# ForeverFancy/GVFDiffusion

Measured on AMD Instinct MI355X. Metric: 4D frames/sec (800x800x24f, 256k Gaussians) + DiT denoise steps/sec, higher is better.
Workload: dtype f32

## Files before the change

gvfdiffusion_amd/csrc/rast.hip:

```cpp
#include <atomic>
#include <cstdlib>
#include <mutex>
#include <vector>
#include "gvf_common.h"
#include "gvf_sort.h"
#include "../../include/gvf_rast.h"

namespace {

constexpr int PRE_THREADS = 256;
constexpr int NSLAB = 1;
#ifndef GVF_PRE_FB
#define GVF_PRE_FB 4
#endif
constexpr int PRE_FB = GVF_PRE_FB;
#ifndef GVF_PRE_XCD
#define GVF_PRE_XCD 0
#endif
#ifndef GVF_PRE_REC_QUAD
#define GVF_PRE_REC_QUAD 1
#endif
#ifndef GVF_PRE_PREFETCH
#define GVF_PRE_PREFETCH 0
#endif
constexpr int TILE = GVF_TILE;
constexpr int BLEND_THREADS = TILE * TILE;
constexpr int MAX_SH_COEFFS = 16;
constexpr float CONIC_K1 = -0.7213475204444817f;
constexpr float CONIC_K2 = -1.4426950408889634f;
constexpr float CONIC_IK1 = -1.3862943611198906f;
constexpr float CONIC_IK2 = -0.6931471805599453f;
struct SplatChol { float l11, l12, l22, c1, c2; bool ok; };
__device__ __forceinline__ SplatChol splat_cholesky(float x, float y, float ap, float bp, float cp, float tile_x0, float tile_y0) {
    SplatChol r;
    const float m11 = -ap, m12 = -0.5f * bp, m22 = -cp;
    const float il = __builtin_amdgcn_rsqf(m11);
    r.l11 = m11 * il;
    r.l12 = m12 * il;
    const float d = m22 - r.l12 * r.l12;
    r.l22 = __builtin_amdgcn_sqrtf(d);
    r.ok = m11 > 0.0f && d > 0.0f && m11 < __builtin_inff() && d < __builtin_inff();
    if (!r.ok) { r.l11 = 0.f; r.l12 = 0.f; r.l22 = 0.f; }
    const float xr = x - tile_x0, yr = y - tile_y0;
    r.c1 = r.ok ? __builtin_fmaf(r.l11, xr, r.l12 * yr) : 0.f;
    r.c2 = r.ok ? r.l22 * yr : 0.f;
    return r;
}
__device__ __forceinline__ float splat_neg_exponent(float l11, float l12, float l22, float c1, float c2, float px, float py, float lo = 0.0f) {
    const float s1 = __builtin_fmaf(-l11, px, __builtin_fmaf(-l12, py, c1));
    const float s2 = __builtin_fmaf(-l22, py, c2);
    return __builtin_fmaf(s2, s2, __builtin_fmaf(s1, s1, -lo));
}

__constant__ float SH_C0 = 0.28209479177387814f;
__constant__ float SH_C1 = 0.4886025119029199f;
__constant__ float SH_C2[5] = {1.0925484305920792f, -1.0925484305920792f, 0.31539156525252005f,
                               -1.0925484305920792f, 0.5462742152960396f};
__constant__ float SH_C3[7] = {-0.5900435899266435f, 2.890611442640554f, -0.4570457994644658f,
                               0.3731763325901154f, -0.4570457994644658f, 1.445305721320277f,
                               -0.5900435899266435f};

struct PreParams {
    int P, M, deg, H, W, mode;
    int gx, gy;
    float kernel_size, scale_modifier;
    int fused;
    GvfGaussianActivation act;
    int n_delta;
    int upstream_binning;
    int F;
};

__device__ __forceinline__ float act_expf(float x) {
    if (x != x) return x;
    if (x > 88.72283f) return __builtin_inff();
    if (x < -103.97208f) return 0.0f;
    const float kf = x * 1.44269502f + (x < 0.0f ? -0.5f : 0.5f);
    const int k = (int)kf;
    const float t = (float)k;
    float r = __builtin_fmaf(t, -0.693145751953125f, x);
    r = __builtin_fmaf(t, -1.42860677e-6f, r);
    float p = 1.98412698e-4f;
    p = __builtin_fmaf(p, r, 1.38888889e-3f);
    p = __builtin_fmaf(p, r, 8.33333377e-3f);
    p = __builtin_fmaf(p, r, 4.16666679e-2f);
    p = __builtin_fmaf(p, r, 1.66666672e-1f);
    p = __builtin_fmaf(p, r, 0.5f);
    p = __builtin_fmaf(p, r, 1.0f);
    p = __builtin_fmaf(p, r, 1.0f);
    const int k1 = k / 2, k2 = k - k1;
    return (p * __uint_as_float((uint32_t)(k1 + 127) << 23)) * __uint_as_float((uint32_t)(k2 + 127) << 23);
}
__device__ __forceinline__ float act_log1pf(float y) {
    if (!(y >= 5.9604645e-8f)) return y;
    if (y > 3.4028235e38f) return y;
    int k = 0;
    float c = 0.0f, f = y;
    if (y >= 0.41421354f) {
        const float u = 1.0f + y;
        uint32_t iu = __float_as_uint(u) + (0x3f800000u - 0x3f3504f3u);
        k = (int)(iu >> 23) - 127;
        if (k < 25) c = (k >= 2 ? 1.0f - (u - y) : y - (u - 1.0f)) / u;
        iu = (iu & 0x007fffffu) + 0x3f3504f3u;
        f = __uint_as_float(iu) - 1.0f;
    }
    const float s = f / (2.0f + f);
    const float z = s * s, w = z * z;
    const float t1 = w * (0.40000972152f + w * 0.24279078841f);
    const float t2 = z * (0.66666662693f + w * 0.28498786688f);
    const float R = t2 + t1;
    const float hfsq = (0.5f * f) * f;
    const float dk = (float)k;
    float acc = s * (hfsq + R);
    acc = acc + (dk * 9.0580006145e-6f + c);
    acc = acc - hfsq;
    acc = acc + f;
    return acc + dk * 6.9313812256e-1f;
}
#ifdef ACT_ABL_LIBM
#define act_expf expf
#define act_log1pf log1pf
#endif
__device__ __forceinline__ float act_scale(float x, const GvfGaussianActivation& a) {
// ... 193 lines not shown
    return make_float2(sqrtf(tau * cc * inv) * 1.001f + 0.01f, sqrtf(tau * ca * inv) * 1.001f + 0.01f);
}

__device__ __forceinline__ void tight_range(float c, float h, int lo, int hi, int n, int& t0, int& t1) {
    if (h < 0.0f) { t0 = lo; t1 = lo; return; }
    const float a = fminf(fmaxf(ceilf((c - h - (float)(TILE - 1)) / (float)TILE), 0.0f), (float)n);
    const float b = fminf(fmaxf(floorf((c + h) / (float)TILE) + 1.0f, 0.0f), (float)n);
    t0 = max((int)a, lo);
    t1 = min((int)b, hi);
    if (t1 < t0) t1 = t0;
}

__device__ __forceinline__ TileRect tight_rect(TileRect r, float px, float py, float hx, float hy, int gx, int gy) {
    TileRect t;
    tight_range(px, hx, r.x0, r.x1, gx, t.x0, t.x1);
    tight_range(py, hy, r.y0, r.y1, gy, t.y0, t.y1);
    return t;
}

template <bool SHARED>
__global__ __launch_bounds__(PRE_THREADS) void preprocess_kernel(
    PreParams pp, const GvfRastFrame* __restrict__ frames, const float* __restrict__ a0,
    const float* __restrict__ a1, const float* __restrict__ a2, const float* __restrict__ a3,
    const float* __restrict__ sh, const float* __restrict__ colors_precomp,
    const float* __restrict__ cov3D_precomp, const float* __restrict__ delta, float4* __restrict__ splats,
    uint32_t* __restrict__ tiles_touched,
    int32_t* __restrict__ radii, uint32_t* __restrict__ block_sums, uint4* __restrict__ binrec,
    const uint32_t* __restrict__ bin_slot ,
    const float2* __restrict__ zrange ) {
    extern __shared__ __attribute__((aligned(16))) float sh_lds[];
    const int t = threadIdx.x;
    const int P = pp.P, M = pp.M;
    const int nbx = (P + PRE_THREADS - 1) / PRE_THREADS;
    int bx = blockIdx.x, by = blockIdx.y;
    if (GVF_PRE_XCD) {
        const int FY = (pp.F + PRE_FB - 1) / PRE_FB, k = (int)(blockIdx.x >> 3);
        bx = (k / FY) * 8 + (int)(blockIdx.x & 7u);
        by = k - (k / FY) * FY;
        if (bx >= nbx) return;
    }
    const int i = bx * PRE_THREADS + t;

    const int sh_stride = M * 3;
    if (sh != nullptr) {
        const size_t span0 = (size_t)bx * PRE_THREADS * sh_stride;
        const int nvalid = min(PRE_THREADS, P - bx * PRE_THREADS);
        const int total = nvalid * sh_stride;
        const float4* src4 = reinterpret_cast<const float4*>(sh + span0);
        float4* dst4 = reinterpret_cast<float4*>(sh_lds);
        const int n4 = total >> 2;
        for (int k = t; k < n4; k += PRE_THREADS) dst4[k] = src4[k];
        for (int k = (n4 << 2) + t; k < total; k += PRE_THREADS) sh_lds[k] = sh[span0 + k];
    }
    __syncthreads();

  const uint32_t my_slot = (bin_slot != nullptr && i < P) ? bin_slot[i] : (uint32_t)i;
#if GVF_PRE_PREFETCH
  float dnx[14];
  bool dnx_has = false;
  auto fetch_delta = [&](int f_) {
      dnx_has = false;
      if (pp.fused && delta != nullptr && i < P && f_ < pp.F) {
          const int di = frames[f_].delta_index;
          if (di >= 0) {
              const float* d = delta + ((size_t)di * P + i) * 14;
#pragma unroll
              for (int k = 0; k < 14; ++k) dnx[k] = d[k];
              dnx_has = true;
          }
      }
      if (!dnx_has) {
#pragma unroll
          for (int k = 0; k < 14; ++k) dnx[k] = 0.0f;
      }
  };
  fetch_delta(by * PRE_FB);
#endif
  for (int ff = 0; ff < PRE_FB; ++ff) {
    const int f = by * PRE_FB + ff;
    if (f >= pp.F) break;
    const GvfRastFrame* fr = frames + f;
#if GVF_PRE_PREFETCH
    float dcur[14];
#pragma unroll
    for (int k = 0; k < 14; ++k) dcur[k] = dnx[k];
    const bool dcur_has = dnx_has;
    if (ff + 1 < PRE_FB) fetch_delta(f + 1);
#endif
    uint32_t touched = 0;
    int radius_out = 0;
    float4 gA = make_float4(0.f, 0.f, 0.f, 0.f), gB = gA, gC = gA;
    TileRect rect = {0, 0, 0, 0};

    if (i < P) {
        float p[3], s[3], q[4], op, dadd[3] = {0.f, 0.f, 0.f};
        float c6s[6];
        if (SHARED) {
            const float4* r3 = reinterpret_cast<const float4*>(a0) + 4 * ((size_t)fr->reserved[0] * P + i);
            const float4 r0 = r3[0], r1 = r3[1], r2 = r3[2], r3v = r3[3];
            p[0] = r0.x; p[1] = r0.y; p[2] = r0.z; op = r0.w;
            c6s[0] = r1.x; c6s[1] = r1.y; c6s[2] = r1.z; c6s[3] = r1.w; c6s[4] = r2.x; c6s[5] = r2.y;
            dadd[0] = r2.z; dadd[1] = r2.w; dadd[2] = r3v.x;
        } else if (pp.fused) {
#if GVF_PRE_PREFETCH
            ActGaussian g = activate_vals(i, pp.act, a0, a1, a2, a3, dcur, dcur_has);
#else
            const int di = fr->delta_index;
            const float* d = (delta != nullptr && di >= 0) ? delta + ((size_t)di * P + i) * 14 : nullptr;
            ActGaussian g = activate_one(i, pp.act, a0, a1, a2, a3, d);
#endif
#pragma unroll
            for (int k = 0; k < 3; ++k) { p[k] = g.p[k]; s[k] = g.s[k]; dadd[k] = g.drgb[k]; }
#pragma unroll
            for (int k = 0; k < 4; ++k) q[k] = g.q[k];
            op = g.op;
        } else {
#pragma unroll
            for (int k = 0; k < 3; ++k) p[k] = a0[3 * (size_t)i + k];
            if (cov3D_precomp == nullptr) {
#pragma unroll
                for (int k = 0; k < 3; ++k) s[k] = a1[3 * (size_t)i + k];
#pragma unroll
                for (int k = 0; k < 4; ++k) q[k] = a2[4 * (size_t)i + k];
            }
            op = a3[i];
        }

        float pv[3];
        xform43(fr->viewmatrix, p, pv);
        bool vis = pv[2] > 0.2f;
        if (vis) {
            float ph[4];
            xform44(fr->projmatrix, p, ph);
            float pw = 1.0f / (ph[3] + 0.0000001f);
            float projx = ph[0] * pw, projy = ph[1] * pw;

            float c6[6];
            if (SHARED) {
#pragma unroll
                for (int k = 0; k < 6; ++k) c6[k] = c6s[k];
            } else if (!pp.fused && cov3D_precomp != nullptr) {
#pragma unroll
                for (int k = 0; k < 6; ++k) c6[k] = cov3D_precomp[6 * (size_t)i + k];
            } else {
                cov3d_from_scale_rot(s, pp.scale_modifier, q, c6);
            }

            const float tanfovx = fr->tanfovx, tanfovy = fr->tanfovy;
            float focal_x = (float)pp.W / (2.0f * tanfovx);
            float focal_y = (float)pp.H / (2.0f * tanfovy);
            float limx = 1.3f * tanfovx, limy = 1.3f * tanfovy;
            float txtz = pv[0] / pv[2], tytz = pv[1] / pv[2];
            float tx = fminf(limx, fmaxf(-limx, txtz)) * pv[2];
            float ty = fminf(limy, fmaxf(-limy, tytz)) * pv[2];
            float tz = pv[2];
            float J00 = focal_x / tz, J02 = -(focal_x * tx) / (tz * tz);
            float J11 = focal_y / tz, J12 = -(focal_y * ty) / (tz * tz);
            float A0[3], A1[3];
// ... 15 lines not shown
            float cyy = B1[0] * A1[0] + B1[1] * A1[1] + B1[2] * A1[2];

            float coef = 1.0f;
            if (pp.mode == GVF_RAST_MODE_MIP) {
                float det0 = fmaxf(1e-6f, cxx * cyy - cxy * cxy);
                float det1 = fmaxf(1e-6f, (cxx + pp.kernel_size) * (cyy + pp.kernel_size) - cxy * cxy);
                coef = sqrtf(det0 / (det1 + 1e-6f) + 1e-6f);
                if (det0 <= 1e-6f || det1 <= 1e-6f) coef = 0.0f;
                cxx += pp.kernel_size;
                cyy += pp.kernel_size;
            } else {
                cxx += 0.3f;
                cyy += 0.3f;
            }
            float det = cxx * cyy - cxy * cxy;
            if (det != 0.0f) {
                float det_inv = 1.f / det;
                float ca = cyy * det_inv, cb = -cxy * det_inv, cc = cxx * det_inv;
                float mid = 0.5f * (cxx + cyy);
                float lam1 = mid + sqrtf(fmaxf(0.1f, mid * mid - det));
                float lam2 = mid - sqrtf(fmaxf(0.1f, mid * mid - det));
                float my_radius = ceilf(3.f * sqrtf(fmaxf(lam1, lam2)));
                float px = ((projx + 1.0f) * (float)pp.W - 1.0f) * 0.5f;
                float py = ((projy + 1.0f) * (float)pp.H - 1.0f) * 0.5f;
                TileRect r = get_rect(px, py, my_radius, pp.gx, pp.gy);
                uint32_t cnt = (uint32_t)((r.x1 - r.x0) * (r.y1 - r.y0));
                if (cnt != 0) {
                    float rgb[3];
                    if (colors_precomp != nullptr) {
                        rgb[0] = colors_precomp[3 * (size_t)i + 0];
                        rgb[1] = colors_precomp[3 * (size_t)i + 1];
                        rgb[2] = colors_precomp[3 * (size_t)i + 2];
                    } else {
                        sh_to_rgb(pp.deg, sh_lds + t * sh_stride, dadd, p, fr->campos, rgb);
                    }
                    radius_out = (int)my_radius;
                    const float2 ext = cull_extent(ca, cb, cc, op * coef);
                    if (!pp.upstream_binning) {
                        r = tight_rect(r, px, py, ext.x, ext.y, pp.gx, pp.gy);
                        cnt = (uint32_t)((r.x1 - r.x0) * (r.y1 - r.y0));
                    }
                    touched = cnt;
                    rect = r;
                    gA = make_float4(px, py, ca * CONIC_K1, cb * CONIC_K2);
                    gB = make_float4(cc * CONIC_K1, op * coef, rgb[0], rgb[1]);
                    gC = make_float4(rgb[2], pv[2], ext.x, ext.y);
                }
            }
        }
        const size_t o = (size_t)f * P + i;
#if defined(PRE_ABL_NOREC)
        if (touched != 0 && gA.x == 12345.678f) splats[4 * o] = gA;
#else
        if (!(GVF_PRE_REC_QUAD && SHARED) && touched != 0) {
            float4* rec = splats + 4 * o;
            rec[0] = gA; rec[1] = gB; rec[2] = gC;
        }
#endif
        if (tiles_touched != nullptr) tiles_touched[o] = touched;
        if (radii != nullptr) {
            const uint32_t* gid_of = SHARED ? reinterpret_cast<const uint32_t*>(a1) : nullptr;
            radii[gid_of != nullptr ? (size_t)f * P + gid_of[i] : o] = radius_out;
        }
        if (binrec != nullptr) {
            uint32_t slab = 0u;
            if (zrange != nullptr) {
                const float2 zr = zrange[f];
                slab = (uint32_t)fminf(fmaxf((gC.y - zr.x) * zr.y, 0.0f), (float)(NSLAB - 1));
            }
#if defined(PRE_ABL_NOBIN)
            if (gC.y == 12345.678f)
#elif defined(PRE_ABL_BINLINEAR)
            binrec[(size_t)f * P + i] = make_uint4((uint32_t)rect.x0 | ((uint32_t)rect.y0 << 16), (uint32_t)rect.x1 | ((uint32_t)rect.y1 << 16), __float_as_uint(gC.y), slab);
            if (false)
#endif
            binrec[(size_t)f * P + my_slot] = make_uint4((uint32_t)rect.x0 | ((uint32_t)rect.y0 << 16),
                                                         (uint32_t)rect.x1 | ((uint32_t)rect.y1 << 16), __float_as_uint(gC.y), slab);
        }
    }

#if !defined(PRE_ABL_NOREC)
    if (GVF_PRE_REC_QUAD && SHARED) {
        const int lj = t & 3;
        float4* qbase = splats + 4 * ((size_t)f * P + (size_t)(i & ~3));
#define GVF_QB(v_, k_) __builtin_bit_cast(float, __builtin_amdgcn_mov_dpp(__builtin_bit_cast(int, (v_)), (k_) * 0x55, 0xF, 0xF, true))
#define GVF_QSTORE(k_)                                                                                          \
        {                                                                                                       \
            const int tk = __builtin_amdgcn_mov_dpp((int)touched, (k_) * 0x55, 0xF, 0xF, true);                 \
            float4 o4;                                                                                          \
            { const float a = GVF_QB(gA.x, k_), b = GVF_QB(gB.x, k_), c = GVF_QB(gC.x, k_); o4.x = lj == 0 ? a : (lj == 1 ? b : (lj == 2 ? c : 0.f)); } \
            { const float a = GVF_QB(gA.y, k_), b = GVF_QB(gB.y, k_), c = GVF_QB(gC.y, k_); o4.y = lj == 0 ? a : (lj == 1 ? b : (lj == 2 ? c : 0.f)); } \
            { const float a = GVF_QB(gA.z, k_), b = GVF_QB(gB.z, k_), c = GVF_QB(gC.z, k_); o4.z = lj == 0 ? a : (lj == 1 ? b : (lj == 2 ? c : 0.f)); } \
            { const float a = GVF_QB(gA.w, k_), b = GVF_QB(gB.w, k_), c = GVF_QB(gC.w, k_); o4.w = lj == 0 ? a : (lj == 1 ? b : (lj == 2 ? c : 0.f)); } \
            if (tk != 0) qbase[4 * (k_) + lj] = o4;                                                             \
        }
        GVF_QSTORE(0) GVF_QSTORE(1) GVF_QSTORE(2) GVF_QSTORE(3)
#undef GVF_QSTORE
#undef GVF_QB
    }
#endif

    if (block_sums != nullptr) {
        const unsigned lane = t & 63, w = t >> 6;
        uint32_t incl = gvf_wave_incl_scan(touched, lane);
        __shared__ uint32_t wsum[PRE_THREADS / GVF_WAVE];
        __syncthreads();
        if (lane == 63) wsum[w] = incl;
        __syncthreads();
        if (t == 0) block_sums[(size_t)f * nbx + bx] = wsum[0] + wsum[1] + wsum[2] + wsum[3];
    }
  }
}

__global__ __launch_bounds__(1024) void scan_sums_kernel(uint32_t* __restrict__ block_sums, int nb, int F,
                                                         uint32_t* __restrict__ frame_base ,
                                                         uint32_t* __restrict__ num_rendered ,
                                                         uint32_t* __restrict__ total_out, uint32_t max_rendered) {
    __shared__ uint32_t wsum[16];
    __shared__ uint32_t carry_s;
    const int t = threadIdx.x;
    const unsigned lane = t & 63, w = t >> 6;
    const int n = nb * F;
    if (t == 0) carry_s = 0;
    __syncthreads();
    for (int base = 0; base < n; base += 1024) {
        int j = base + t;
        uint32_t v = j < n ? block_sums[j] : 0u;
        uint32_t incl = gvf_wave_incl_scan(v, lane);
        if (lane == 63) wsum[w] = incl;
        __syncthreads();
        uint32_t wbase = 0, tot = 0;
        for (unsigned k = 0; k < 16; ++k) { if (k < w) wbase += wsum[k]; tot += wsum[k]; }
        uint32_t carry = carry_s;
        uint32_t excl = carry + wbase + incl - v;
        if (j < n) {
            block_sums[j] = excl;
            if (j % nb == 0) frame_base[j / nb] = excl;
        }
        __syncthreads();
        if (t == 0) carry_s = carry + tot;
        __syncthreads();
    }
    if (t == 0) { frame_base[F] = carry_s; *total_out = carry_s > max_rendered ? 0u : carry_s; }
    __syncthreads();
    for (int f = t; f < F; f += 1024) num_rendered[f] = frame_base[f + 1] - frame_base[f];
}

__global__ __launch_bounds__(PRE_THREADS) void duplicate_kernel(
    int P, int gx, int gy, const float4* __restrict__ splats,
    const uint32_t* __restrict__ tiles_touched, const int32_t* __restrict__ radii_ws,
    const uint32_t* __restrict__ block_base, uint64_t* __restrict__ keys, uint32_t* __restrict__ vals,
    uint32_t max_rendered, int upstream_binning) {
    __shared__ uint32_t wsum[PRE_THREADS / GVF_WAVE];
    const int t = threadIdx.x, f = blockIdx.y;
    const int i = blockIdx.x * PRE_THREADS + t;
    const unsigned lane = t & 63, w = t >> 6;
    const size_t o = (size_t)f * P + i;
    uint32_t touched = i < P ? tiles_touched[o] : 0u;
    uint32_t incl = gvf_wave_incl_scan(touched, lane);
    if (lane == 63) wsum[w] = incl;
    __syncthreads();
    uint32_t wbase = 0;
    for (unsigned k = 0; k < w; ++k) wbase += wsum[k];
// ... 90 lines not shown
        if (j < n) {
            ranges[j] = overflow ? make_uint2(0u, 0u) : make_uint2(run, run + c[k]);
            cursor[j] = run;
            if (!overflow && c[k] > (uint32_t)SORT_SMALL_N) {
                if (c[k] > (uint32_t)SORT_LARGE_N) cls[2 + n + atomicAdd(&cls[1], 1u)] = (uint32_t)j;
                else cls[2 + atomicAdd(&cls[0], 1u)] = (uint32_t)j | (c[k] > (uint32_t)SORT_MEDIUM_N ? 0x80000000u : 0u);
            }
            if (j % per_frame == 0) frame_base[j / per_frame] = run;
        }
        run += c[k];
    }
    if (blockIdx.x == 0 && t == 0) { frame_base[F] = total; *total_out = overflow ? 0u : total; }
}

__global__ void frame_counts_kernel(const uint32_t* __restrict__ frame_base, int F, uint32_t* __restrict__ num_rendered) {
    const int f = blockIdx.x * blockDim.x + threadIdx.x;
    if (f < F) num_rendered[f] = frame_base[f + 1] - frame_base[f];
}

__global__ void frame_zrange_kernel(const GvfRastFrame* __restrict__ frames, int F, const uint32_t* __restrict__ mm,
                                    int fused, GvfGaussianActivation act, float2* __restrict__ zrange) {
    const int f = blockIdx.x * blockDim.x + threadIdx.x;
    if (f >= F) return;
    float lo[3], hi[3];
#pragma unroll
    for (int k = 0; k < 3; ++k) {
        lo[k] = float_unordered(mm[k]); hi[k] = float_unordered(mm[3 + k]);
        if (fused) { lo[k] = lo[k] * act.aabb[3 + k] + act.aabb[k]; hi[k] = hi[k] * act.aabb[3 + k] + act.aabb[k]; }
        if (lo[k] > hi[k]) { const float tmp = lo[k]; lo[k] = hi[k]; hi[k] = tmp; }
    }
    const float* V = frames[f].viewmatrix;
    float zmin = 3.0e38f, zmax = -3.0e38f;
    for (int c = 0; c < 8; ++c) {
        const float p[3] = {(c & 1) ? hi[0] : lo[0], (c & 2) ? hi[1] : lo[1], (c & 4) ? hi[2] : lo[2]};
        const float z = V[2] * p[0] + V[6] * p[1] + V[10] * p[2] + V[14];
        zmin = fminf(zmin, z); zmax = fmaxf(zmax, z);
    }
    zmin = fmaxf(zmin, 0.2f);
    const float ext = fmaxf(zmax - zmin, 1e-6f);
    zrange[f] = make_float2(zmin - 0.02f * ext, (float)NSLAB / (1.04f * ext));
}

constexpr int WIN_MAX = 2048;
constexpr int BIN_SPT = 4;
constexpr int BIN_SLOTS = PRE_THREADS * BIN_SPT;

template <bool SCATTER>
__global__ __launch_bounds__(PRE_THREADS) void bin_kernel(int P, int gx, int gy, const uint4* __restrict__ binrec,
                                                          const uint32_t* __restrict__ order,
                                                          uint32_t* __restrict__ tile_count ,
                                                          uint32_t* __restrict__ cursor ,
                                                          const uint32_t* __restrict__ total,
                                                          uint64_t* __restrict__ payload, int nslab,
                                                          const uint32_t* __restrict__ frame_base, uint32_t* __restrict__ num_rendered) {
    __shared__ uint32_t s_tab[WIN_MAX];
    __shared__ uint32_t s_run[SCATTER ? WIN_MAX : 1];
    __shared__ int s_box[4];
    if (SCATTER && num_rendered != nullptr && blockIdx.x == 0 && threadIdx.x == 0)
        num_rendered[blockIdx.y] = frame_base[blockIdx.y + 1] - frame_base[blockIdx.y];
    if (SCATTER && *total == 0u) return;
    const int t = threadIdx.x, lane = t & 63, f = blockIdx.y;
    if (t == 0) { s_box[0] = 0x7fffffff; s_box[1] = 0x7fffffff; s_box[2] = 0; s_box[3] = 0; }
    int x0[BIN_SPT], y0[BIN_SPT], x1[BIN_SPT], y1[BIN_SPT], sl[BIN_SPT];
    uint64_t key[BIN_SPT];
    int bx0 = 0x7fffffff, by0 = 0x7fffffff, bx1 = 0, by1 = 0;
#pragma unroll
    for (int k = 0; k < BIN_SPT; ++k) {
        const int s = blockIdx.x * BIN_SLOTS + k * PRE_THREADS + t;
        x0[k] = y0[k] = x1[k] = y1[k] = 0; sl[k] = 0; key[k] = 0;
        if (s < P) {
            const uint32_t id = order != nullptr ? order[s] : (uint32_t)s;
            const uint4 br = binrec[(size_t)f * P + s];
            x0[k] = (int)(br.x & 0xffffu); y0[k] = (int)(br.x >> 16);
            x1[k] = (int)(br.y & 0xffffu); y1[k] = (int)(br.y >> 16);
            sl[k] = (int)br.w;
            key[k] = ((uint64_t)br.z << 32) | id;
            if (x1[k] > x0[k] && y1[k] > y0[k]) {
                bx0 = min(bx0, x0[k]); by0 = min(by0, y0[k]); bx1 = max(bx1, x1[k]); by1 = max(by1, y1[k]);
            } else {
                x1[k] = x0[k];
            }
        }
    }
#pragma unroll
    for (int d = 32; d >= 1; d >>= 1) {
        bx0 = min(bx0, __shfl_xor(bx0, d, 64)); by0 = min(by0, __shfl_xor(by0, d, 64));
        bx1 = max(bx1, __shfl_xor(bx1, d, 64)); by1 = max(by1, __shfl_xor(by1, d, 64));
    }
    __syncthreads();
    if (lane == 0 && bx1 > bx0) {
        atomicMin(&s_box[0], bx0); atomicMin(&s_box[1], by0); atomicMax(&s_box[2], bx1); atomicMax(&s_box[3], by1);
    }
    __syncthreads();
    const int wx0 = s_box[0], wy0 = s_box[1], ww = s_box[2] - s_box[0], wh = s_box[3] - s_box[1];
    if (ww <= 0 || wh <= 0) return;
    uint32_t* gtab = (SCATTER ? cursor : tile_count) + (size_t)f * gx * gy * nslab;
    if (ww * wh * nslab <= WIN_MAX) {
        const int area = ww * wh * nslab;
        for (int e = t; e < area; e += PRE_THREADS) { s_tab[e] = 0u; if (SCATTER) s_run[e] = 0u; }
        __syncthreads();
#pragma unroll
        for (int k = 0; k < BIN_SPT; ++k)
            for (int y = y0[k]; y < y1[k]; ++y)
                for (int x = x0[k]; x < x1[k]; ++x) atomicAdd(&s_tab[((y - wy0) * ww + (x - wx0)) * nslab + sl[k]], 1u);
        __syncthreads();
        for (int e = t; e < area; e += PRE_THREADS) {
            const uint32_t c = s_tab[e];
            if (c != 0u) {
                const int wt = e / nslab;
                const int seg = ((wy0 + wt / ww) * gx + wx0 + wt % ww) * nslab + (e - wt * nslab);
                if (SCATTER) s_tab[e] = atomicAdd(&gtab[seg], c);
                else atomicAdd(&gtab[seg], c);
            }
        }
        if (SCATTER) {
            __syncthreads();
#pragma unroll
            for (int k = 0; k < BIN_SPT; ++k)
                for (int y = y0[k]; y < y1[k]; ++y)
                    for (int x = x0[k]; x < x1[k]; ++x) {
                        const int e = ((y - wy0) * ww + (x - wx0)) * nslab + sl[k];
                        payload[s_tab[e] + atomicAdd(&s_run[e], 1u)] = key[k];
                    }
        }
    } else {
#pragma unroll
        for (int k = 0; k < BIN_SPT; ++k)
            for (int y = y0[k]; y < y1[k]; ++y)
                for (int x = x0[k]; x < x1[k]; ++x) {
                    const uint32_t pos = atomicAdd(&gtab[(y * gx + x) * nslab + sl[k]], 1u);
                    if (SCATTER) payload[pos] = key[k];
                }
    }
}

__global__ __launch_bounds__(256) void bbox_kernel(int P, const float* __restrict__ xyz, uint32_t* __restrict__ mm) {
    __shared__ uint32_t s_mm[6];
    if (threadIdx.x < 6) s_mm[threadIdx.x] = threadIdx.x < 3 ? 0xffffffffu : 0u;
    __syncthreads();
    uint32_t lo[3] = {0xffffffffu, 0xffffffffu, 0xffffffffu}, hi[3] = {0u, 0u, 0u};
    for (int i = blockIdx.x * blockDim.x + threadIdx.x; i < P; i += gridDim.x * blockDim.x) {
#pragma unroll
        for (int k = 0; k < 3; ++k) {
            const float v = xyz[3 * (size_t)i + k];
            if (v == v && fabsf(v) < 3.0e38f) {
                const uint32_t o = float_ordered(v);
                lo[k] = min(lo[k], o); hi[k] = max(hi[k], o);
            }
        }
    }
#pragma unroll
    for (int k = 0; k < 3; ++k) {
#pragma unroll
        for (int d = 32; d >= 1; d >>= 1) {
            lo[k] = min(lo[k], (uint32_t)__shfl_xor((int)lo[k], d, 64));
            hi[k] = max(hi[k], (uint32_t)__shfl_xor((int)hi[k], d, 64));
        }
        if ((threadIdx.x & 63) == 0) { atomicMin(&s_mm[k], lo[k]); atomicMax(&s_mm[3 + k], hi[k]); }
    }
    __syncthreads();
    if (threadIdx.x < 3) atomicMin(&mm[threadIdx.x], s_mm[threadIdx.x]);
    else if (threadIdx.x < 6) atomicMax(&mm[threadIdx.x], s_mm[threadIdx.x]);
}

__device__ __forceinline__ uint32_t spread5(uint32_t v) {
    return (v & 1u) | ((v & 2u) << 2) | ((v & 4u) << 4) | ((v & 8u) << 6) | ((v & 16u) << 8);
}

constexpr int MORTON_BINS = 1 << 15;

__device__ __forceinline__ uint32_t morton15(int i, const float* __restrict__ xyz, const uint32_t* __restrict__ mm) {
    uint32_t code = 0;
#pragma unroll
    for (int k = 0; k < 3; ++k) {
        const float lo = float_unordered(mm[k]), hi = float_unordered(mm[3 + k]);
        const float v = xyz[3 * (size_t)i + k];
        float q = (v - lo) / fmaxf(hi - lo, 1e-30f) * 32.0f;
        q = (q == q) ? fminf(fmaxf(q, 0.0f), 31.0f) : 0.0f;
        code |= spread5((uint32_t)q) << k;
    }
    return code;
}

__global__ __launch_bounds__(256) void morton_count_kernel(int P, const float* __restrict__ xyz,
                                                           const uint32_t* __restrict__ mm, uint32_t* __restrict__ codes,
// ... 777 lines not shown
    w.frame_base = c.take<uint32_t>(F + 1);
    w.total = c.take<uint32_t>(1);
    w.keys = c.take<uint64_t>(D);
    w.keys_alt = c.take<uint64_t>(D);
    w.vals = c.take<uint32_t>(D);
    w.vals_alt = c.take<uint32_t>(D);
    w.ids = c.take<uint32_t>(D);
    w.ranges = c.take<uint2>((size_t)F * ntiles * NSLAB);
    w.cls = c.take<uint32_t>(2 + 2 * (size_t)F * ntiles * NSLAB);
    w.tile_count = c.take<uint32_t>((size_t)F * ntiles * NSLAB);
    w.cursor = c.take<uint32_t>((size_t)F * ntiles * NSLAB);
    w.partial = c.take<uint32_t>(((size_t)F * ntiles * NSLAB + SCAN_CHUNK - 1) / SCAN_CHUNK + 1);
    w.zrange = c.take<float2>(F);
    const size_t Pp = (size_t)(P > 0 ? P : 1);
    w.order = c.take<uint32_t>(Pp);
    w.order_alt = c.take<uint32_t>(Pp);
    w.mhist = c.take<uint32_t>(1 << 15);
    w.mm = c.take<uint32_t>(8);
    w.binrec = c.take<uint4>(FP);
    w.sort_tmp_bytes = gvf_sort_tmp_bytes((int64_t)D);
    w.sort_tmp = c.take<char>(w.sort_tmp_bytes);
    w.bytes = gvf_align_up(c.off, 256);
    w.ok = c.ok;
    return w;
}

std::atomic<long long> g_shared_calls{0};

int run_pipeline(const GvfRastSettings& st, const GvfRastFrame* frames_host, int F, int P, int M, bool fused,
                 const GvfGaussianActivation* act, const float* a0, const float* a1, const float* a2,
                 const float* a3, const float* sh, const float* colors_precomp, const float* cov3D_precomp,
                 const float* delta, int n_delta, const float* subpixel_offset, void* workspace,
                 size_t workspace_bytes, int64_t max_rendered, float* out_color, float* out_alpha,
                 float* out_depth, int32_t* out_radii, uint32_t* out_num_rendered, hipStream_t stream,
                 unsigned char* out_u8 = nullptr ) {
    const int H = st.image_height, W = st.image_width;
    if (H <= 0 || W <= 0 || P < 0 || F <= 0 || max_rendered < 0 || max_rendered > 0xFFFFFFFFll) return GVF_EINVAL;
    if (st.sh_degree < 0 || st.sh_degree > 3) return GVF_EINVAL;
    if (st.mode != GVF_RAST_MODE_MIP && st.mode != GVF_RAST_MODE_DILATE) return GVF_EINVAL;
    if ((out_color == nullptr) == (out_u8 == nullptr) || !out_num_rendered || !frames_host || !workspace) return GVF_EINVAL;
    if (P > 0 && colors_precomp == nullptr) {
        if (sh == nullptr || M < (st.sh_degree + 1) * (st.sh_degree + 1) || M > MAX_SH_COEFFS) return GVF_EINVAL;
    }
    (void)hipGetLastError();
    if ((((uintptr_t)sh) & 15) != 0 || (((uintptr_t)workspace) & 255) != 0) return GVF_EINVAL;
    Workspace w = carve(workspace, workspace_bytes, P, F, H, W, max_rendered);
    if (!w.ok) return GVF_ENOSPC;

    const int gx = (W + TILE - 1) / TILE, gy = (H + TILE - 1) / TILE, ntiles = gx * gy;
    const int nb = (P + PRE_THREADS - 1) / PRE_THREADS;
    int slot = g_prof.on ? g_prof.calls.fetch_add(1) : -1;
    if (slot >= PROF_MAX_CALLS) slot = -1;

    const bool morton = st.bin_algo != GVF_RAST_BIN_RADIX && F >= 4 && P >= 4096;
    ActSlices slices; slices.n = 0;
    bool shared = false;
    std::vector<int> frame_slice((size_t)F, 0);
    const char* shared_env = getenv("GVF_RAST_SHARED_ACT");
    const bool shared_on = !(shared_env && shared_env[0] == '0');
    if (shared_on && fused && cov3D_precomp == nullptr && st.bin_algo != GVF_RAST_BIN_RADIX && P > 0 && F >= 2) {
        shared = true;
        for (int f = 0; f < F && shared; ++f) {
            const int di = (delta != nullptr && frames_host[f].delta_index >= 0) ? frames_host[f].delta_index : -1;
            int k = 0;
            while (k < slices.n && slices.di[k] != di) ++k;
            if (k == slices.n) {
                if (slices.n == ACT_MAX_SLICES) { shared = false; break; }
                slices.di[slices.n++] = di;
            }
            frame_slice[(size_t)f] = k;
        }
        if (shared && (F < 2 * slices.n || (size_t)slices.n * (size_t)P * 64u > (size_t)(max_rendered > 0 ? max_rendered : 0) * 8u)) shared = false;
    }
    for (int f0 = 0; f0 < F; f0 += 16) {
        FrameChunk ch;
        const int cnt = F - f0 < 16 ? F - f0 : 16;
        for (int k = 0; k < cnt; ++k) {
            ch.f[k] = frames_host[f0 + k];
            ch.f[k].reserved[0] = shared ? frame_slice[(size_t)(f0 + k)] : 0;
        }
        CallTables tab = {};
        if (f0 == 0) {
            const size_t nseg_all = (size_t)F * ntiles * NSLAB;
            tab.ranges = reinterpret_cast<uint32_t*>(w.ranges); tab.n_ranges = (uint32_t)(2 * nseg_all);
            tab.tile_count = w.tile_count; tab.n_tile_count = (uint32_t)nseg_all;
            tab.mhist = w.mhist; tab.n_mhist = morton ? (uint32_t)MORTON_BINS : 0u;
            tab.cls = w.cls; tab.mm = w.mm;
        }
        const size_t clear_words = (size_t)tab.n_ranges + tab.n_tile_count + tab.n_mhist;
        const int zb = f0 == 0 ? (int)((clear_words + 4095) / 4096 < 256 ? (clear_words + 4095) / 4096 : 256) : 0;
        hipLaunchKernelGGL(upload_frames_kernel, dim3(1 + zb), dim3(256), 0, stream, ch, cnt, w.frames + f0, tab);
    }
    GVF_CHECK_LAUNCH();

    int nslab_blend = 1;
    const uint32_t* blend_rec_of = nullptr;
    if (P == 0 || nb == 0) {
        if (hipMemsetAsync(out_num_rendered, 0, sizeof(uint32_t) * F, stream) != hipSuccess) return GVF_ELAUNCH;
    } else {
        const bool bucket = st.bin_algo != GVF_RAST_BIN_RADIX;
        prof_mark(stream, slot, 0);
        const uint32_t* order = nullptr;
        if (morton) {
            int bb = (P + 255) / 256; if (bb > 128) bb = 128;
            const int pb = (P + 255) / 256;
            hipLaunchKernelGGL(bbox_kernel, dim3(bb), dim3(256), 0, stream, P, a0, w.mm);
            hipLaunchKernelGGL(morton_count_kernel, dim3(pb), dim3(256), 0, stream, P, a0, w.mm, w.order_alt, w.mhist);
            hipLaunchKernelGGL(morton_scan_kernel, dim3(1), dim3(1024), 0, stream, w.mhist);
            hipLaunchKernelGGL(morton_scatter_kernel, dim3(pb), dim3(256), 0, stream, P, w.order_alt, w.mhist, w.order);
            order = w.order;
            if (NSLAB > 1)
                hipLaunchKernelGGL(frame_zrange_kernel, dim3((F + 63) / 64), dim3(64), 0, stream, w.frames, F, w.mm, fused ? 1 : 0,
                                   fused ? *act : GvfGaussianActivation{}, w.zrange);
            GVF_CHECK_LAUNCH();
        }
        const int nslab = order != nullptr ? NSLAB : 1;
        nslab_blend = nslab;
        const unsigned nseg = (unsigned)((size_t)F * ntiles * nslab);
        prof_mark(stream, slot, 1);
        PreParams pp;
        pp.P = P; pp.M = colors_precomp ? 0 : M; pp.deg = st.sh_degree; pp.H = H; pp.W = W; pp.mode = st.mode;
        pp.gx = gx; pp.gy = gy; pp.kernel_size = st.kernel_size; pp.scale_modifier = st.scale_modifier;
        pp.fused = fused ? 1 : 0; pp.n_delta = n_delta; pp.F = F;
        pp.upstream_binning = (st.upstream_binning != 0 || subpixel_offset != nullptr) ? 1 : 0;
        if (fused) pp.act = *act; else pp.act = GvfGaussianActivation{};
        const size_t sh_lds_bytes = gvf_align_up((size_t)PRE_THREADS * pp.M * 3 * sizeof(float), 16) + 16;
        const int pre_fy = (F + PRE_FB - 1) / PRE_FB;
        const dim3 pre_grid = GVF_PRE_XCD ? dim3((nb + 7) / 8 * 8 * pre_fy) : dim3(nb, pre_fy);
        if (shared) {
            g_shared_calls.fetch_add(1, std::memory_order_relaxed);
            float4* rec3d = reinterpret_cast<float4*>(w.keys_alt);
            const char* slot_env = getenv("GVF_RAST_SLOT_ORDER");
            const size_t sh_floats = (size_t)pp.M * 3;
            const bool slot_mode = !(slot_env && slot_env[0] == '0') && order != nullptr && colors_precomp == nullptr && sh != nullptr &&
                                   (size_t)slices.n * (size_t)P * 64u + (size_t)P * sh_floats * 4u <= (size_t)max_rendered * 8u;
            float* sh_by_slot = slot_mode ? reinterpret_cast<float*>(rec3d + 4 * (size_t)slices.n * (size_t)P) : nullptr;
            hipLaunchKernelGGL(activate_cov_kernel, dim3((P + 255) / 256, slices.n), dim3(256), 0, stream, *act, st.scale_modifier, P, slices,
                               a0, a1, a2, a3, delta, rec3d, slot_mode ? w.order_alt : nullptr, sh, (int)sh_floats, sh_by_slot);
            if (slot_mode) {
                blend_rec_of = w.order_alt;
                hipLaunchKernelGGL(preprocess_kernel<true>, pre_grid, dim3(PRE_THREADS), sh_lds_bytes, stream, pp,
                                   w.frames, reinterpret_cast<const float*>(rec3d), reinterpret_cast<const float*>(order), nullptr, nullptr, sh_by_slot,
                                   nullptr, nullptr, nullptr, w.splats, nullptr, out_radii == nullptr ? nullptr : w.radii, nullptr, w.binrec,
                                   nullptr, nslab > 1 ? w.zrange : nullptr);
            } else
            hipLaunchKernelGGL(preprocess_kernel<true>, pre_grid, dim3(PRE_THREADS), sh_lds_bytes, stream, pp,
                               w.frames, reinterpret_cast<const float*>(rec3d), nullptr, nullptr, nullptr, colors_precomp ? nullptr : sh, colors_precomp,
                               nullptr, nullptr, w.splats, nullptr, out_radii == nullptr ? nullptr : w.radii, nullptr, w.binrec,
                               order != nullptr ? w.order_alt : nullptr, nslab > 1 ? w.zrange : nullptr);
        } else
        hipLaunchKernelGGL(preprocess_kernel<false>, pre_grid, dim3(PRE_THREADS), sh_lds_bytes, stream, pp,
                           w.frames, a0, a1, a2, a3, colors_precomp ? nullptr : sh, colors_precomp, cov3D_precomp, delta,
                           w.splats, bucket ? nullptr : w.tiles_touched, (bucket && out_radii == nullptr) ? nullptr : w.radii,
                           bucket ? nullptr : w.block_sums, bucket ? w.binrec : nullptr, order != nullptr ? w.order_alt : nullptr,
                           (bucket && nslab > 1) ? w.zrange : nullptr);
        const int bnb = (P + BIN_SLOTS - 1) / BIN_SLOTS;
        if (bucket)
            hipLaunchKernelGGL(bin_kernel<false>, dim3(bnb, F), dim3(PRE_THREADS), 0, stream, P, gx, gy, w.binrec, order,
                               w.tile_count, w.cursor, w.total, w.keys, nslab, nullptr, nullptr);
        GVF_CHECK_LAUNCH();
        prof_mark(stream, slot, 2);
        if (bucket)
        {
            const int sblocks = (int)((nseg + SCAN_CHUNK - 1) / SCAN_CHUNK);
            hipLaunchKernelGGL(seg_sums_kernel, dim3(sblocks), dim3(1024), 0, stream, w.tile_count, (int)nseg, w.partial);
            hipLaunchKernelGGL(seg_scan_kernel, dim3(sblocks), dim3(1024), 0, stream, w.tile_count, (int)nseg, ntiles * nslab, F,
                               w.partial, sblocks, w.ranges, w.cursor, w.frame_base, out_num_rendered, w.total,
                               (uint32_t)max_rendered, w.cls);
            if (max_rendered <= 0)
                hipLaunchKernelGGL(frame_counts_kernel, dim3((F + 63) / 64), dim3(64), 0, stream, w.frame_base, F, out_num_rendered);
        }
        else
            hipLaunchKernelGGL(scan_sums_kernel, dim3(1), dim3(1024), 0, stream, w.block_sums, nb, F, w.frame_base,
                               out_num_rendered, w.total, (uint32_t)max_rendered);
        GVF_CHECK_LAUNCH();
        prof_mark(stream, slot, 3);
        if (max_rendered > 0) {
            if (bucket)
                hipLaunchKernelGGL(bin_kernel<true>, dim3(bnb, F), dim3(PRE_THREADS), 0, stream, P, gx, gy, w.binrec, order,
                                   w.tile_count, w.cursor, w.total, w.keys, nslab, w.frame_base, out_num_rendered);
            else
                hipLaunchKernelGGL(duplicate_kernel, dim3(nb, F), dim3(PRE_THREADS), 0, stream, P, gx, gy, w.splats,
                                   w.tiles_touched, w.radii, w.block_sums, w.keys, w.vals, (uint32_t)max_rendered,
                                   pp.upstream_binning);
            GVF_CHECK_LAUNCH();
        }
        if (out_radii != nullptr) {
            if (hipMemcpyAsync(out_radii, w.radii, sizeof(int32_t) * (size_t)F * P, hipMemcpyDeviceToDevice, stream) != hipSuccess)
                return GVF_ELAUNCH;
        }
        prof_mark(stream, slot, 4);
        if (max_rendered > 0) {
            uint64_t* keys_sorted = w.keys;
            uint32_t* vals_by_tile = nullptr;
            if (!bucket) {
                vals_by_tile = w.vals;
                int in_alt = 0;
                int rc = gvf_sort_pairs_device_n(w.keys, w.keys_alt, w.vals, w.vals_alt, w.total, max_rendered, 32,
                                                 key_end_bit(F, ntiles), w.sort_tmp, w.sort_tmp_bytes, stream, &in_alt);
                if (rc != GVF_OK) return rc;
                if (in_alt) { keys_sorted = w.keys_alt; vals_by_tile = w.vals_alt; }
                int rblocks = (int)((max_rendered + 255) / 256);
                if (rblocks > 4096) rblocks = 4096;
                hipLaunchKernelGGL(ranges_kernel, dim3(rblocks), dim3(256), 0, stream, keys_sorted, w.total,
                                   (uint32_t)max_rendered, w.ranges, (uint32_t)nseg);
                GVF_CHECK_LAUNCH();
            }
            prof_mark(stream, slot, 5);
            const int rc = launch_tile_sort(stream, w.ranges, keys_sorted, vals_by_tile, w.ids, w.cls, nseg, bucket ? 2 : 1);
            if (rc != GVF_OK) return rc;
        } else {
            prof_mark(stream, slot, 5);
        }
    }
    uint32_t* vals_sorted = w.ids;
    const char* order_env = getenv("GVF_RAST_BLEND_ORDER");
    const uint32_t* tile_order = nullptr;
    if (!(order_env && order_env[0] == '0') && P > 0 && nb > 0 && max_rendered > 0 && nslab_blend == 1 && (size_t)F * ntiles >= 2048) {
        hipLaunchKernelGGL(blend_order_kernel, dim3(F), dim3(1024), 0, stream, w.ranges, ntiles, w.cursor);
        tile_order = w.cursor;
    }
    prof_mark(stream, slot, 6);
    if (out_depth != nullptr)
        hipLaunchKernelGGL(blend_kernel<true>, dim3(ntiles, F), dim3(BLEND_THREADS), 0, stream, P, H, W, gx, gy, st.bg[0],
                           st.bg[1], st.bg[2], w.ranges, vals_sorted, w.splats, subpixel_offset,
                           out_color, out_alpha, out_depth, nslab_blend, tile_order, blend_rec_of, out_u8);
    else
        hipLaunchKernelGGL(blend_kernel<false>, dim3(ntiles, F), dim3(BLEND_THREADS), 0, stream, P, H, W, gx, gy, st.bg[0],
                           st.bg[1], st.bg[2], w.ranges, vals_sorted, w.splats, subpixel_offset,
                           out_color, out_alpha, out_depth, nslab_blend, tile_order, blend_rec_of, out_u8);
    GVF_CHECK_LAUNCH();
    prof_mark(stream, slot, 7);
    return GVF_OK;
// ... 633 lines not shown
```

Measured before the change: 19450.

## Add index-order binning count kernel, gathered binrec reads, and quad record writes

Adds a bin_index_kernel that counts tile coverage per frame using an LDS histogram over large chunks of Gaussians in index order. With the default GVF_BIN_ALGO=2 it replaces the counting pass of bin_kernel when the tile table fits in LDS. For the non-shared path it also reads binrec by Gaussian id instead of by sorted slot (rec_gather) and remaps the bin grid to interleave frames across XCDs. It enables the DPP quad-packed splat record writes for the non-shared preprocess path as well. An optional LDS staging path for delta rows is added but disabled by default. The aim is less global atomic traffic and more coalesced record reads, at the cost of scattered gathers through order[] and more launch-configuration complexity.

Result: faster. 20740 (median of 6 runs) (+6.7%).

```diff
diff --git a/gvfdiffusion_amd/csrc/rast.hip b/gvfdiffusion_amd/csrc/rast.hip
--- a/gvfdiffusion_amd/csrc/rast.hip
+++ b/gvfdiffusion_amd/csrc/rast.hip
@@ -1,6 +1,7 @@
 #include <atomic>
 #include <cstdlib>
 #include <mutex>
+#include <type_traits>
 #include <vector>
 #include "gvf_common.h"
 #include "gvf_sort.h"
@@ -22,6 +23,12 @@
 #endif
 #ifndef GVF_PRE_PREFETCH
 #define GVF_PRE_PREFETCH 0
+#endif
+#ifndef GVF_PRE_DELTA_LDS
+#define GVF_PRE_DELTA_LDS 0
+#endif
+#ifndef GVF_BIN_ALGO
+#define GVF_BIN_ALGO 2
 #endif
 constexpr int TILE = GVF_TILE;
 constexpr int BLEND_THREADS = TILE * TILE;
@@ -69,6 +76,7 @@
     int n_delta;
     int upstream_binning;
     int F;
+    int delta_lds;
 };
 
 __device__ __forceinline__ float act_expf(float x) {
@@ -368,6 +376,31 @@
         for (int k = t; k < n4; k += PRE_THREADS) dst4[k] = src4[k];
         for (int k = (n4 << 2) + t; k < total; k += PRE_THREADS) sh_lds[k] = sh[span0 + k];
     }
+#if GVF_PRE_DELTA_LDS
+    float* d_lds = sh_lds + ((size_t)PRE_THREADS * sh_stride * 4 + 15) / 16 * 4 + 4;
+    const bool dstage = !SHARED && pp.delta_lds && pp.fused && delta != nullptr;
+    const int dq = min(PRE_THREADS, P - bx * PRE_THREADS) * 14 / 4;
+    float4 dreg0 = make_float4(0.f, 0.f, 0.f, 0.f), dreg1 = dreg0, dreg2 = dreg0, dreg3 = dreg0;
+    auto dfetch = [&](int f_) -> bool {
+        const int di_ = frames[f_].delta_index;
+        if (di_ < 0) return false;
+        const float4* src = reinterpret_cast<const float4*>(delta + ((size_t)di_ * P + (size_t)bx * PRE_THREADS) * 14) + t;
+        if (t < dq) dreg0 = src[0];
+        if (t + PRE_THREADS < dq) dreg1 = src[PRE_THREADS];
+        if (t + 2 * PRE_THREADS < dq) dreg2 = src[2 * PRE_THREADS];
+        if (t + 3 * PRE_THREADS < dq) dreg3 = src[3 * PRE_THREADS];
+        return true;
+    };
+    auto dcommit = [&]() {
+        float4* dst = reinterpret_cast<float4*>(d_lds) + t;
+        if (t < dq) dst[0] = dreg0;
+        if (t + PRE_THREADS < dq) dst[PRE_THREADS] = dreg1;
+        if (t + 2 * PRE_THREADS < dq) dst[2 * PRE_THREADS] = dreg2;
+        if (t + 3 * PRE_THREADS < dq) dst[3 * PRE_THREADS] = dreg3;
+    };
+    bool dcur = false;
+    if (dstage && by * PRE_FB < pp.F) { dcur = dfetch(by * PRE_FB); if (dcur) dcommit(); }
+#endif
     __syncthreads();
 
   const uint32_t my_slot = (bin_slot != nullptr && i < P) ? bin_slot[i] : (uint32_t)i;
@@ -396,6 +429,23 @@
     const int f = by * PRE_FB + ff;
     if (f >= pp.F) break;
     const GvfRastFrame* fr = frames + f;
+#if GVF_PRE_DELTA_LDS
+    float drow[14];
+    if (dstage) {
+        if (dcur && i < P) {
+#pragma unroll
+            for (int k = 0; k < 14; ++k) drow[k] = d_lds[t * 14 + k];
+        } else {
+#pragma unroll
+            for (int k = 0; k < 14; ++k) drow[k] = 0.0f;
+        }
+    }
+    bool dnext = false;
+    if (dstage && ff + 1 < PRE_FB && f + 1 < pp.F) {
+        __syncthreads();
+        dnext = dfetch(f + 1);
+    }
+#endif
 #if GVF_PRE_PREFETCH
     float dcur[14];
 #pragma unroll
@@ -420,6 +470,16 @@
         } else if (pp.fused) {
 #if GVF_PRE_PREFETCH
             ActGaussian g = activate_vals(i, pp.act, a0, a1, a2, a3, dcur, dcur_has);
+#elif GVF_PRE_DELTA_LDS
+            bool dhas = dcur;
+            if (!dstage) {
+                const int di = fr->delta_index;
+                const float* d = (delta != nullptr && di >= 0) ? delta + ((size_t)di * P + i) * 14 : nullptr;
+#pragma unroll
+                for (int k = 0; k < 14; ++k) drow[k] = d ? d[k] : 0.0f;
+                dhas = d != nullptr;
+            }
+            ActGaussian g = activate_vals(i, pp.act, a0, a1, a2, a3, drow, dhas);
 #else
             const int di = fr->delta_index;
             const float* d = (delta != nullptr && di >= 0) ? delta + ((size_t)di * P + i) * 14 : nullptr;
@@ -541,7 +601,7 @@
 #if defined(PRE_ABL_NOREC)
         if (touched != 0 && gA.x == 12345.678f) splats[4 * o] = gA;
 #else
-        if (!(GVF_PRE_REC_QUAD && SHARED) && touched != 0) {
+        if (!GVF_PRE_REC_QUAD && touched != 0) {
             float4* rec = splats + 4 * o;
             rec[0] = gA; rec[1] = gB; rec[2] = gC;
         }
@@ -559,9 +619,6 @@
             }
 #if defined(PRE_ABL_NOBIN)
             if (gC.y == 12345.678f)
-#elif defined(PRE_ABL_BINLINEAR)
-            binrec[(size_t)f * P + i] = make_uint4((uint32_t)rect.x0 | ((uint32_t)rect.y0 << 16), (uint32_t)rect.x1 | ((uint32_t)rect.y1 << 16), __float_as_uint(gC.y), slab);
-            if (false)
 #endif
             binrec[(size_t)f * P + my_slot] = make_uint4((uint32_t)rect.x0 | ((uint32_t)rect.y0 << 16),
                                                          (uint32_t)rect.x1 | ((uint32_t)rect.y1 << 16), __float_as_uint(gC.y), slab);
@@ -569,7 +626,7 @@
     }
 
 #if !defined(PRE_ABL_NOREC)
-    if (GVF_PRE_REC_QUAD && SHARED) {
+    if (GVF_PRE_REC_QUAD) {
         const int lj = t & 3;
         float4* qbase = splats + 4 * ((size_t)f * P + (size_t)(i & ~3));
 #define GVF_QB(v_, k_) __builtin_bit_cast(float, __builtin_amdgcn_mov_dpp(__builtin_bit_cast(int, (v_)), (k_) * 0x55, 0xF, 0xF, true))
@@ -598,6 +655,10 @@
         __syncthreads();
         if (t == 0) block_sums[(size_t)f * nbx + bx] = wsum[0] + wsum[1] + wsum[2] + wsum[3];
     }
+#if GVF_PRE_DELTA_LDS
+    if (dnext) { dcommit(); __syncthreads(); }
+    dcur = dnext;
+#endif
   }
 }
 
@@ -794,25 +855,33 @@
                                                           uint32_t* __restrict__ cursor ,
                                                           const uint32_t* __restrict__ total,
                                                           uint64_t* __restrict__ payload, int nslab,
-                                                          const uint32_t* __restrict__ frame_base, uint32_t* __restrict__ num_rendered) {
+                                                          const uint32_t* __restrict__ frame_base, uint32_t* __restrict__ num_rendered,
+                                                          int rec_by_id, int xcd_frames, int F) {
     __shared__ uint32_t s_tab[WIN_MAX];
     __shared__ uint32_t s_run[SCATTER ? WIN_MAX : 1];
     __shared__ int s_box[4];
-    if (SCATTER && num_rendered != nullptr && blockIdx.x == 0 && threadIdx.x == 0)
-        num_rendered[blockIdx.y] = frame_base[blockIdx.y + 1] - frame_base[blockIdx.y];
+    int blk = (int)blockIdx.x, f = (int)blockIdx.y;
+    if (xcd_frames) {
+        const int nblk = (P + BIN_SLOTS - 1) / BIN_SLOTS, k = (int)(blockIdx.x >> 3);
+        f = (k / nblk) * 8 + (int)(blockIdx.x & 7u);
+        blk = k - (k / nblk) * nblk;
+        if (f >= F) return;
+    }
+    if (SCATTER && num_rendered != nullptr && blk == 0 && threadIdx.x == 0)
+        num_rendered[f] = frame_base[f + 1] - frame_base[f];
     if (SCATTER && *total == 0u) return;
-    const int t = threadIdx.x, lane = t & 63, f = blockIdx.y;
+    const int t = threadIdx.x, lane = t & 63;
     if (t == 0) { s_box[0] = 0x7fffffff; s_box[1] = 0x7fffffff; s_box[2] = 0; s_box[3] = 0; }
     int x0[BIN_SPT], y0[BIN_SPT], x1[BIN_SPT], y1[BIN_SPT], sl[BIN_SPT];
     uint64_t key[BIN_SPT];
     int bx0 = 0x7fffffff, by0 = 0x7fffffff, bx1 = 0, by1 = 0;
 #pragma unroll
     for (int k = 0; k < BIN_SPT; ++k) {
-        const int s = blockIdx.x * BIN_SLOTS + k * PRE_THREADS + t;
+        const int s = blk * BIN_SLOTS + k * PRE_THREADS + t;
         x0[k] = y0[k] = x1[k] = y1[k] = 0; sl[k] = 0; key[k] = 0;
         if (s < P) {
             const uint32_t id = order != nullptr ? order[s] : (uint32_t)s;
-            const uint4 br = binrec[(size_t)f * P + s];
+            const uint4 br = binrec[(size_t)f * P + (rec_by_id ? id : (uint32_t)s)];
             x0[k] = (int)(br.x & 0xffffu); y0[k] = (int)(br.x >> 16);
             x1[k] = (int)(br.y & 0xffffu); y1[k] = (int)(br.y >> 16);
             sl[k] = (int)br.w;
@@ -873,6 +942,66 @@
                     const uint32_t pos = atomicAdd(&gtab[(y * gx + x) * nslab + sl[k]], 1u);
                     if (SCATTER) payload[pos] = key[k];
                 }
+    }
+}
+
+constexpr int BINX_THREADS = 512;
+constexpr int BINX_TAB = 4096;
+constexpr int BINX_PER_WG = 8192;
+constexpr int BINX_SPT = 4;
+
+template <bool SCATTER>
+__global__ __launch_bounds__(BINX_THREADS) void bin_index_kernel(int P, int gx, const uint4* __restrict__ binrec,
+                                                                 uint32_t* __restrict__ tile_count ,
+                                                                 uint32_t* __restrict__ cursor ,
+                                                                 const uint32_t* __restrict__ total,
+                                                                 uint64_t* __restrict__ payload, int nslab, int nseg_frame,
+                                                                 const uint32_t* __restrict__ frame_base, uint32_t* __restrict__ num_rendered) {
+    __shared__ uint32_t s_tab[BINX_TAB];
+    __shared__ uint32_t s_run[SCATTER ? BINX_TAB : 1];
+    const int t = threadIdx.x, f = blockIdx.y;
+    if (SCATTER && num_rendered != nullptr && blockIdx.x == 0 && t == 0) num_rendered[f] = frame_base[f + 1] - frame_base[f];
+    if (SCATTER && *total == 0u) return;
+    const int g0 = (int)blockIdx.x * BINX_PER_WG, g1 = min(P, g0 + BINX_PER_WG);
+    const uint4* rec = binrec + (size_t)f * P;
+    for (int e = t; e < nseg_frame; e += BINX_THREADS) { s_tab[e] = 0u; if (SCATTER) s_run[e] = 0u; }
+    __syncthreads();
+    auto sweep = [&](auto pass) {
+        for (int base = g0; base < g1; base += BINX_SPT * BINX_THREADS) {
+            uint4 br[BINX_SPT];
+#pragma unroll
+            for (int k = 0; k < BINX_SPT; ++k) {
+                const int s = base + k * BINX_THREADS + t;
+                br[k] = s < g1 ? rec[s] : make_uint4(0u, 0u, 0u, 0u);
+            }
+#pragma unroll
+            for (int k = 0; k < BINX_SPT; ++k) {
+                const int x0 = (int)(br[k].x & 0xffffu), y0 = (int)(br[k].x >> 16);
+                const int x1 = (int)(br[k].y & 0xffffu), y1 = (int)(br[k].y >> 16);
+                const int sl = (int)br[k].w;
+                const uint64_t key = ((uint64_t)br[k].z << 32) | (uint32_t)(base + k * BINX_THREADS + t);
+                for (int y = y0; y < y1; ++y)
+                    for (int x = x0; x < x1; ++x) {
+                        const int e = (y * gx + x) * nslab + sl;
+                        if constexpr (decltype(pass)::value == 0) atomicAdd(&s_tab[e], 1u);
+                        else payload[s_tab[e] + atomicAdd(&s_run[e], 1u)] = key;
+                    }
+            }
+        }
+    };
+    sweep(std::integral_constant<int, 0>{});
+    __syncthreads();
+    uint32_t* gtab = (SCATTER ? cursor : tile_count) + (size_t)f * nseg_frame;
+    for (int e = t; e < nseg_frame; e += BINX_THREADS) {
+        const uint32_t c = s_tab[e];
+        if (c != 0u) {
+            if (SCATTER) s_tab[e] = atomicAdd(&gtab[e], c);
+            else atomicAdd(&gtab[e], c);
+        }
+    }
+    if (SCATTER) {
+        __syncthreads();
+        sweep(std::integral_constant<int, 1>{});
     }
 }
 
@@ -1756,7 +1885,6 @@
     int slot = g_prof.on ? g_prof.calls.fetch_add(1) : -1;
     if (slot >= PROF_MAX_CALLS) slot = -1;
 
-    const bool morton = st.bin_algo != GVF_RAST_BIN_RADIX && F >= 4 && P >= 4096;
     ActSlices slices; slices.n = 0;
     bool shared = false;
     std::vector<int> frame_slice((size_t)F, 0);
@@ -1776,6 +1904,9 @@
         }
         if (shared && (F < 2 * slices.n || (size_t)slices.n * (size_t)P * 64u > (size_t)(max_rendered > 0 ? max_rendered : 0) * 8u)) shared = false;
     }
+    const bool index_fits = st.bin_algo != GVF_RAST_BIN_RADIX && !shared && (size_t)ntiles * NSLAB <= (size_t)BINX_TAB;
+    const bool index_count = GVF_BIN_ALGO >= 2 && index_fits, index_scatter = GVF_BIN_ALGO == 3 && index_fits;
+    const bool morton = st.bin_algo != GVF_RAST_BIN_RADIX && F >= 4 && P >= 4096 && !index_scatter;
     for (int f0 = 0; f0 < F; f0 += 16) {
         FrameChunk ch;
         const int cnt = F - f0 < 16 ? F - f0 : 16;
@@ -1819,6 +1950,7 @@
             GVF_CHECK_LAUNCH();
         }
         const int nslab = order != nullptr ? NSLAB : 1;
+        const bool rec_gather = GVF_BIN_ALGO >= 1 && bucket && !shared && order != nullptr;
         nslab_blend = nslab;
         const unsigned nseg = (unsigned)((size_t)F * ntiles * nslab);
         prof_mark(stream, slot, 1);
@@ -1829,6 +1961,8 @@
         pp.upstream_binning = (st.upstream_binning != 0 || subpixel_offset != nullptr) ? 1 : 0;
         if (fused) pp.act = *act; else pp.act = GvfGaussianActivation{};
         const size_t sh_lds_bytes = gvf_align_up((size_t)PRE_THREADS * pp.M * 3 * sizeof(float), 16) + 16;
+        pp.delta_lds = (GVF_PRE_DELTA_LDS && fused && delta != nullptr && P % 2 == 0 && (((uintptr_t)delta) & 15) == 0) ? 1 : 0;
+        const size_t pre_lds_bytes = sh_lds_bytes + (pp.delta_lds ? (size_t)PRE_THREADS * 14 * sizeof(float) : 0);
         const int pre_fy = (F + PRE_FB - 1) / PRE_FB;
         const dim3 pre_grid = GVF_PRE_XCD ? dim3((nb + 7) / 8 * 8 * pre_fy) : dim3(nb, pre_fy);
         if (shared) {
@@ -1853,15 +1987,19 @@
                                nullptr, nullptr, w.splats, nullptr, out_radii == nullptr ? nullptr : w.radii, nullptr, w.binrec,
                                order != nullptr ? w.order_alt : nullptr, nslab > 1 ? w.zrange : nullptr);
         } else
-        hipLaunchKernelGGL(preprocess_kernel<false>, pre_grid, dim3(PRE_THREADS), sh_lds_bytes, stream, pp,
+        hipLaunchKernelGGL(preprocess_kernel<false>, pre_grid, dim3(PRE_THREADS), pre_lds_bytes, stream, pp,
                            w.frames, a0, a1, a2, a3, colors_precomp ? nullptr : sh, colors_precomp, cov3D_precomp, delta,
                            w.splats, bucket ? nullptr : w.tiles_touched, (bucket && out_radii == nullptr) ? nullptr : w.radii,
-                           bucket ? nullptr : w.block_sums, bucket ? w.binrec : nullptr, order != nullptr ? w.order_alt : nullptr,
-                           (bucket && nslab > 1) ? w.zrange : nullptr);
-        const int bnb = (P + BIN_SLOTS - 1) / BIN_SLOTS;
-        if (bucket)
-            hipLaunchKernelGGL(bin_kernel<false>, dim3(bnb, F), dim3(PRE_THREADS), 0, stream, P, gx, gy, w.binrec, order,
-                               w.tile_count, w.cursor, w.total, w.keys, nslab, nullptr, nullptr);
+                           bucket ? nullptr : w.block_sums, bucket ? w.binrec : nullptr,
+                           (order != nullptr && !rec_gather) ? w.order_alt : nullptr, (bucket && nslab > 1) ? w.zrange : nullptr);
+        const int bnb = (P + BIN_SLOTS - 1) / BIN_SLOTS, xnb = (P + BINX_PER_WG - 1) / BINX_PER_WG;
+        const dim3 bin_grid = rec_gather ? dim3((unsigned)((F + 7) / 8 * 8 * bnb)) : dim3(bnb, F);
+        if (index_count)
+            hipLaunchKernelGGL(bin_index_kernel<false>, dim3(xnb, F), dim3(BINX_THREADS), 0, stream, P, gx, w.binrec,
+                               w.tile_count, w.cursor, w.total, w.keys, nslab, ntiles * nslab, nullptr, nullptr);
+        else if (bucket)
+            hipLaunchKernelGGL(bin_kernel<false>, bin_grid, dim3(PRE_THREADS), 0, stream, P, gx, gy, w.binrec, order,
+                               w.tile_count, w.cursor, w.total, w.keys, nslab, nullptr, nullptr, rec_gather ? 1 : 0, rec_gather ? 1 : 0, F);
         GVF_CHECK_LAUNCH();
         prof_mark(stream, slot, 2);
         if (bucket)
@@ -1880,9 +2018,13 @@
         GVF_CHECK_LAUNCH();
         prof_mark(stream, slot, 3);
         if (max_rendered > 0) {
-            if (bucket)
-                hipLaunchKernelGGL(bin_kernel<true>, dim3(bnb, F), dim3(PRE_THREADS), 0, stream, P, gx, gy, w.binrec, order,
-                                   w.tile_count, w.cursor, w.total, w.keys, nslab, w.frame_base, out_num_rendered);
+            if (index_scatter)
+                hipLaunchKernelGGL(bin_index_kernel<true>, dim3(xnb, F), dim3(BINX_THREADS), 0, stream, P, gx, w.binrec,
+                                   w.tile_count, w.cursor, w.total, w.keys, nslab, ntiles * nslab, w.frame_base, out_num_rendered);
+            else if (bucket)
+                hipLaunchKernelGGL(bin_kernel<true>, bin_grid, dim3(PRE_THREADS), 0, stream, P, gx, gy, w.binrec, order,
+                                   w.tile_count, w.cursor, w.total, w.keys, nslab, w.frame_base, out_num_rendered,
+                                   rec_gather ? 1 : 0, rec_gather ? 1 : 0, F);
             else
                 hipLaunchKernelGGL(duplicate_kernel, dim3(nb, F), dim3(PRE_THREADS), 0, stream, P, gx, gy, w.splats,
                                    w.tiles_touched, w.radii, w.block_sums, w.keys, w.vals, (uint32_t)max_rendered,
```
